# chao1224/GeoSSL

Measured on AMD Instinct MI355X. Metric: molecules/s/GPU SchNet+DDM fwd+bwd (QM9-sized, bs=1024); % HBM roofline, higher is better.
Workload: dtype f32

## Files before the change

### geossl_amd/csrc/ddm.hip

```cpp
#include "common.h"
#include "geossl_hip.h"
#include "tn.h"
#include "wgrad.h"

using namespace geossl;

namespace {

inline int grid1d(int64_t n, int block, int cap = 2048) {
  int64_t g = (n + block - 1) / block;
  return (int)(g < 1 ? 1 : (g > cap ? cap : g));
}

__global__ __launch_bounds__(256) void k_sum_partial(const float* __restrict__ x, int64_t n, float* __restrict__ partial) {
  __shared__ float red[256];
  const int64_t per = (n + gridDim.x - 1) / gridDim.x;
  const int64_t lo = blockIdx.x * per, hi = min(n, lo + per);
  float s = 0.0f;
  for (int64_t i = lo + threadIdx.x; i < hi; i += 256) s += x[i];
  red[threadIdx.x] = s;
  __syncthreads();
  for (int o = 128; o > 0; o >>= 1) {
    if (threadIdx.x < o) red[threadIdx.x] += red[threadIdx.x + o];
    __syncthreads();
  }
  if (threadIdx.x == 0) partial[blockIdx.x] = red[0];
}
__global__ void k_loss_final(const float* __restrict__ partial, int nblk, const int64_t* __restrict__ divisor,
                             float out_scale, float* __restrict__ loss, int accumulate) {
  if (blockIdx.x != 0) return;
  float s = 0.0f;
  for (int b = threadIdx.x; b < nblk; b += 64) s += partial[b];
  s = wave_sum(s);
  if (threadIdx.x != 0) return;
// ... 140 lines not shown
    P[H + F + k] = s_w1;
    P[H + 2 * F + k] = s_b1;
  }
  if (threadIdx.x == 0) {
    float sg = 0.0f, sd = 0.0f;
    for (int s = lo; s < hi; ++s) {
      sg += grow[s];
      sd += demb[s];
    }
    P[H + 3 * F] = sg;
    P[H + 3 * F + 1] = sd;
  }
}
__global__ __launch_bounds__(64) void k_ncsn_small_reduce(const float* __restrict__ partial, int nblk, int F,
                                                          GeosslNcsnGrads g, int accumulate) {
  const int H = F / 2, len = H + 3 * F + 2;
  const int i = blockIdx.x;
  if (i >= len) return;
  float s = 0.0f;
  for (int b = threadIdx.x; b < nblk; b += 64) s += partial[(size_t)b * len + i];
  s = wave_sum(s);
  if (threadIdx.x == 0) {
    float* dst;
    if (i < H) dst = g.o3_w + i;
    else if (i < H + F) dst = g.in_w2 + (i - H);
    else if (i < H + 2 * F) dst = g.in_w1 + (i - H - F);
    else if (i < H + 3 * F) dst = g.in_b1 + (i - H - 2 * F);
    else if (i == H + 3 * F) dst = g.o3_b;
    else dst = g.in_b2;
    *dst = accumulate ? *dst + s : s;
  }
}

__global__ __launch_bounds__(256) void k_incidence_gather(const float* __restrict__ dfeat0,
                                                          const int64_t* __restrict__ inc_ptr,
                                                          const int32_t* __restrict__ inc_idx, int N, int F,
                                                          float* __restrict__ dh0, int accumulate,
                                                          const float* __restrict__ dfeat1, float* __restrict__ dh1,
                                                          const int32_t* __restrict__ dyn_view) {
  const float* __restrict__ dfeat = blockIdx.y == 0 ? dfeat0 : dfeat1;
  float* __restrict__ dh = blockIdx.y == 0 ? dh0 : dh1;
  N = dyn_count(N, dyn_view);
  if (dyn_view != nullptr && blockIdx.y == 1) dh += (size_t)N * F;
  const int per = ((int)gridDim.x + 7) / 8;
  const int grp = ((int)blockIdx.x % 8) * per + (int)blockIdx.x / 8;
  const int a = grp * 4 + (threadIdx.x >> 6), lane = threadIdx.x & 63;
  if (a >= N) return;
  const int64_t p0 = inc_ptr[a], p1 = inc_ptr[a + 1];
  float acc[4] = {0.0f, 0.0f, 0.0f, 0.0f};
  if (accumulate) {
#pragma unroll
    for (int v = 0; v < 4; ++v)
      if (lane + 64 * v < F) acc[v] = dh[(size_t)a * F + lane + 64 * v];
  }
  for (int64_t pb = p0; pb < p1; pb += 64) {
    const int cnt = (int)min((int64_t)64, p1 - pb);
    const int mine = lane < cnt ? inc_idx[pb + lane] : 0;
    for (int q0 = 0; q0 < cnt; q0 += 8) {
      float val[8][4];
#pragma unroll
      for (int u = 0; u < 8; ++u) {
        const int s = __shfl(mine, min(q0 + u, cnt - 1), 64);
#pragma unroll
        for (int v = 0; v < 4; ++v)
          if (lane + 64 * v < F) val[u][v] = dfeat[(size_t)s * F + lane + 64 * v];
      }
#pragma unroll
      for (int u = 0; u < 8; ++u)
        if (q0 + u < cnt) {
#pragma unroll
          for (int v = 0; v < 4; ++v)
            if (lane + 64 * v < F) acc[v] += val[u][v];
        }
    }
  }
#pragma unroll
  for (int v = 0; v < 4; ++v)
    if (lane + 64 * v < F) dh[(size_t)a * F + lane + 64 * v] = acc[v];
}

__global__ void k_adam(float* __restrict__ p, const float* __restrict__ g, float* __restrict__ m,
                       float* __restrict__ v, int64_t n, float step_size, float w1, float beta2, float w2, float eps,
                       float wd, float bc2_sqrt, float grad_scale) {
  for (int64_t i = (int64_t)blockIdx.x * blockDim.x + threadIdx.x; i < n; i += (int64_t)gridDim.x * blockDim.x) {
    float gi = mul_rn(g[i], grad_scale);
    const float pi = p[i];
    if (wd != 0.0f) gi = fmaf(wd, pi, gi);
    const float m0 = m[i];
    const float mi = fmaf(w1, add_rn(gi, -m0), m0);
    const float vi = fmaf(w2, mul_rn(gi, gi), mul_rn(v[i], beta2));
    m[i] = mi;
    v[i] = vi;
    const float denom = add_rn(sqrtf(vi) / bc2_sqrt, eps);
    p[i] = fmaf(-step_size, mi / denom, pi);
  }
}

}

namespace geossl {
int launch_ncsn_small_reduce(const float* partial, int nblk, int F, const GeosslNcsnGrads& g, int accumulate,
                             hipStream_t stream);
}

extern "C" int64_t geossl_loss_reduce_workspace_floats(int64_t S) { return GEOSSL_LOSS_BLOCKS; }

extern "C" int geossl_loss_reduce(const float* loss_e, int64_t S, const int64_t* stats_divisor, float out_scale,
                                  float* loss, float* workspace, int accumulate, hipStream_t stream) {
  hipLaunchKernelGGL(k_sum_partial, dim3(GEOSSL_LOSS_BLOCKS), dim3(256), 0, stream, loss_e, S, workspace);
  GEOSSL_CHECK_LAUNCH();
  hipLaunchKernelGGL(k_loss_final, dim3(1), dim3(64), 0, stream, workspace, GEOSSL_LOSS_BLOCKS, stats_divisor, out_scale,
// ... 47 lines not shown
  NcsnW2Ops l2{grow, w->o3_w, saved->a2, saved->a1, F, H};
  if (F == 128) rc = launch_wgrad_split<2, 4>(l2, 1, S, H, F, o, F, 1, workspace, accumulate, stream);
  else if (F == 64) rc = launch_wgrad_split<1, 2>(l2, 1, S, H, F, o, F, 1, workspace, accumulate, stream);
  else rc = launch_wgrad_split<1, 1>(l2, 1, S, H, F, o, F, 1, workspace, accumulate, stream);
  if (rc) return rc;
  o.dW[0] = grads->o1_w;
  o.db[0] = grads->o1_b;
  o.dd[0] = grads->o1_w + F;
  NcsnW1Ops l1{dz1, h, sei0, sei1, saved->emb, F};
  if (F == 128) rc = launch_wgrad_split<4, 4>(l1, 1, S, F, F, o, F + 1, F + 1, workspace, accumulate, stream);
  else if (F == 64) rc = launch_wgrad_split<2, 2>(l1, 1, S, F, F, o, F + 1, F + 1, workspace, accumulate, stream);
  else rc = launch_wgrad_split<1, 1>(l1, 1, S, F, F, o, F + 1, F + 1, workspace, accumulate, stream);
  if (rc) return rc;
  int chunk, nblk;
  small_plan(S, &chunk, &nblk);
  hipLaunchKernelGGL(k_ncsn_small_partial, dim3(nblk), dim3(128), 0, stream, *w, *saved, grow, demb, (int)S, F, chunk,
                     workspace);
  GEOSSL_CHECK_LAUNCH();
  return launch_ncsn_small_reduce(workspace, nblk, F, *grads, accumulate, stream);
}

namespace geossl {
int launch_ncsn_small_reduce(const float* partial, int nblk, int F, const GeosslNcsnGrads& g, int accumulate,
                             hipStream_t stream) {
  hipLaunchKernelGGL(k_ncsn_small_reduce, dim3(F / 2 + 3 * F + 2), dim3(64), 0, stream, partial, nblk, F, g, accumulate);
  GEOSSL_CHECK_LAUNCH();
  return 0;
}
}

extern "C" int geossl_incidence_gather(const float* dfeat, const int64_t* inc_ptr, const int32_t* inc_idx, int64_t N,
                                       int F, float* dh, int accumulate, hipStream_t stream) {
  if (N <= 0) return 0;
  const unsigned groups = (unsigned)((N + 3) / 4);
  hipLaunchKernelGGL(k_incidence_gather, dim3((groups + 7) / 8 * 8), dim3(256), 0, stream, dfeat, inc_ptr, inc_idx,
                     (int)N, F, dh, accumulate, (const float*)nullptr, (float*)nullptr, (const int32_t*)nullptr);
  GEOSSL_CHECK_LAUNCH();
  return 0;
}

namespace geossl {
int launch_incidence_gather2(const float* dfeat0, const float* dfeat1, const int64_t* inc_ptr, const int32_t* inc_idx,
                             int64_t N, int F, float* dh0, float* dh1, hipStream_t stream, const int32_t* dyn_view) {
  if (N <= 0) return 0;
  const unsigned groups = (unsigned)((N + 3) / 4);
  hipLaunchKernelGGL(k_incidence_gather, dim3((groups + 7) / 8 * 8, 2), dim3(256), 0, stream, dfeat0, inc_ptr, inc_idx,
                     (int)N, F, dh0, 0, dfeat1, dh1, dyn_view);
  GEOSSL_CHECK_LAUNCH();
  return 0;
}
}

extern "C" int geossl_adam_step(float* param, const float* grad, float* exp_avg, float* exp_avg_sq, int64_t n, double lr,
                                double beta1, double beta2, double eps, double weight_decay, int64_t step_count,
                                float grad_scale, hipStream_t stream) {
  if (n <= 0) return 0;
  const double bc1 = 1.0 - pow(beta1, (double)step_count);
  const double bc2 = 1.0 - pow(beta2, (double)step_count);
  hipLaunchKernelGGL(k_adam, dim3(grid1d(n, 256)), dim3(256), 0, stream, param, grad, exp_avg, exp_avg_sq, n,
                     (float)(lr / bc1), (float)(1.0 - beta1), (float)beta2, (float)(1.0 - beta2), (float)eps,
                     (float)weight_decay, (float)sqrt(bc2), grad_scale);
  GEOSSL_CHECK_LAUNCH();
  return 0;
}
```

### geossl_amd/csrc/ncsn_bwd.hip

```cpp
#include "common.h"
#include "geossl_hip.h"
#include "split.h"
#include "tn.h"

using namespace geossl;

namespace {

constexpr int TR = 32;

#ifdef NB_TIMING
__device__ long long nb_dbg[2 * 32 * 8];
#define NB_MARK(slot)                                                                              \
  do {                                                                                             \
    if (blockIdx.x == 5 && lane == 0 && (wave == 0 || wave == NW) && t - t_begin < 32)             \
      nb_dbg[((wave == 0 ? 0 : 1) * 32 + (t - t_begin)) * 8 + (slot)] = clock64();                 \
  } while (0)
#else
#define NB_MARK(slot) do {} while (0)
#endif

template <int NW>
struct NbLds {
  static constexpr int F = 32 * NW, H = F / 2, KHS = (H + 15) / 16, HMB = (H + 31) / 32, KS = F / 16;
  u32x4* zb;
  u32x4* dz2T;
  u32x4* fT;
  u32x4* dz1r;
  u32x4* abT;
  int4* scal;
  float* pdv;
  float* dep;
  float* wls;
  int* eg;
// ... 569 lines not shown
    if (nb < KHS) {
      float* Ps = a.psm + pb * (H + 3 * F + 2);
#pragma unroll
      for (int e = 0; e < 8; ++e) {
        float v = o3acc[e];
#pragma unroll
        for (int o = 16; o > 0; o >>= 1) v += __shfl_xor(v, o, 64);
        const int m = 16 * nb + 8 * kh + e;
        if (j == 0 && m < H) Ps[m] = v;
      }
    }
  }
}

template <int NW>
__global__ __launch_bounds__(128 * NW) void k_ncsn_bwd_fused(NcsnFusedArgs a) {
  if ((int)(threadIdx.x >> 6) < NW) ncsn_bwd_body<NW, true>(a, a.S, a.h);
  else ncsn_bwd_body<NW, false>(a, a.S, a.h);
}
struct NcsnFusedPair { NcsnFusedArgs a[2]; };
template <int NW>
__global__ __launch_bounds__(128 * NW) void k_ncsn_bwd_fused2(NcsnFusedPair pr, const int32_t* __restrict__ dyn_S,
                                                              const int32_t* __restrict__ dyn_view) {
  const NcsnFusedArgs& a = pr.a[blockIdx.y];
  const int S = dyn_count(a.S, dyn_S);
  const float* h = a.h;
  if (dyn_view != nullptr && blockIdx.y == 1) h += (size_t)(*dyn_view) * (32 * NW);
  if ((int)(threadIdx.x >> 6) < NW) ncsn_bwd_body<NW, true>(a, S, h);
  else ncsn_bwd_body<NW, false>(a, S, h);
}

__device__ __forceinline__ void ncsn_reduce_all_block(const ReduceMulti& m, int nblk, int accumulate,
                                                      const float* __restrict__ psm, int F, const GeosslNcsnGrads& g,
                                                      float (*red)[64]) {
  const int mb = m.xoff[m.nseg];
  if ((int)blockIdx.x < mb) {
    reduce_multi_block(m, nblk, accumulate, red, 0);
    return;
  }
  const int H = F / 2, len = H + 3 * F + 2;
  const int i = ((int)blockIdx.x - mb) * 4 + (int)(threadIdx.x >> 6), lane = threadIdx.x & 63;
  if (i >= len) return;
  float s = 0.0f;
  for (int b = lane; b < nblk; b += 64) s += psm[(size_t)b * len + i];
  s = wave_sum(s);
  if (lane == 0) {
    float* dst;
    if (i < H) dst = g.o3_w + i;
    else if (i < H + F) dst = g.in_w2 + (i - H);
    else if (i < H + 2 * F) dst = g.in_w1 + (i - H - F);
    else if (i < H + 3 * F) dst = g.in_b1 + (i - H - 2 * F);
    else if (i == H + 3 * F) dst = g.o3_b;
    else dst = g.in_b2;
    *dst = accumulate ? *dst + s : s;
  }
}
__global__ __launch_bounds__(256) void k_ncsn_reduce_all(ReduceMulti m, int nblk, int accumulate,
                                                         const float* __restrict__ psm, int F, GeosslNcsnGrads g) {
  __shared__ float red[4][64];
  ncsn_reduce_all_block(m, nblk, accumulate, psm, F, g, red);
}
__global__ __launch_bounds__(256) void k_ncsn_reduce_all2(ReduceMulti m0, ReduceMulti m1, int nblk, int accumulate,
                                                          const float* __restrict__ psm0,
                                                          const float* __restrict__ psm1, int F, GeosslNcsnGrads g0,
                                                          GeosslNcsnGrads g1) {
  __shared__ float red[4][64];
  if (blockIdx.y == 0) ncsn_reduce_all_block(m0, nblk, accumulate, psm0, F, g0, red);
  else ncsn_reduce_all_block(m1, nblk, accumulate, psm1, F, g1, red);
}

inline int fused_blocks(int64_t S) {
  const int64_t ntiles = (S + TR - 1) / TR;
  return (int)(ntiles < 256 ? ntiles : 256);
}

}

#ifdef NB_TIMING
extern "C" int geossl_ncsn_bwd_debug_read(long long* host) {
  return (int)hipMemcpyFromSymbol(host, HIP_SYMBOL(nb_dbg), sizeof(long long) * 2 * 32 * 8);
}
#endif

extern "C" int64_t geossl_ddm_loss_bwd_fused_workspace_floats(int64_t S, int F) {
  const int64_t nb = fused_blocks(S), H = F / 2;
  return nb * ((int64_t)F * F + 2 * F + H * F + H + (H + 3 * F + 2));
}

extern "C" int geossl_ddm_loss_bwd_fused(const float* h, const int64_t* sei0, const int64_t* sei1, int64_t S, int64_t N,
                                         int F, const GeosslNcsnWeights* w, const GeosslNcsnSaved* saved,
                                         const int64_t* stats_divisor, float out_scale, const float* gout, float* dfeat,
                                         float* demb, float* grow, const GeosslNcsnGrads* grads, float* workspace,
                                         int accumulate, hipStream_t stream) {
  if (S <= 0) return 0;
  if (F != 32 && F != 64 && F != 128) return (int)hipErrorInvalidValue;
  if (S * (int64_t)F * 4 >= ((int64_t)1 << 32) || N * (int64_t)F * 4 >= ((int64_t)1 << 32)) return (int)hipErrorInvalidValue;
  const int nb = fused_blocks(S), H = F / 2;
  NcsnFusedArgs a;
  a.h = h; a.sei0 = sei0; a.sei1 = sei1; a.S = (int)S; a.w = *w; a.sv = *saved; a.divisor = stats_divisor;
  a.out_scale = out_scale; a.gout = gout; a.dfeat = dfeat; a.demb = demb; a.grow = grow;
  a.pw1 = workspace;
  a.pd1 = a.pw1 + (size_t)nb * F * F;
  a.pb1 = a.pd1 + (size_t)nb * F;
  a.pw2 = a.pb1 + (size_t)nb * F;
  a.pb2 = a.pw2 + (size_t)nb * H * F;
  a.psm = a.pb2 + (size_t)nb * H;
#define LAUNCH(NWV)                                                                                      \
  do {                                                                                                   \
    allow_big_lds(&k_ncsn_bwd_fused<NWV>);                                                               \
    hipLaunchKernelGGL((k_ncsn_bwd_fused<NWV>), dim3(nb), dim3(128 * NWV), NbLds<NWV>::bytes(), stream, a); \
  } while (0)
  if (F == 128) LAUNCH(4); else if (F == 64) LAUNCH(2); else LAUNCH(1);
#undef LAUNCH
  GEOSSL_CHECK_LAUNCH();
  ReduceMulti rm;
  float* o1w[1] = {grads->o1_w};
  float* o1c[1] = {grads->o1_w + F};
  float* o1b[1] = {grads->o1_b};
  float* o2w[1] = {grads->o2_w};
  float* o2b[1] = {grads->o2_b};
  rm.add(a.pw1, F * F, F, F + 1, 1, o1w, 1);
  rm.add(a.pd1, F, F, F, F + 1, o1c, 1);
  rm.add(a.pb1, F, F, F, 1, o1b, 1);
  rm.add(a.pw2, H * F, F, F, 1, o2w, 1);
  rm.add(a.pb2, H, H, H, 1, o2b, 1);
  hipLaunchKernelGGL(k_ncsn_reduce_all, dim3(rm.blocks() + (H + 3 * F + 2 + 3) / 4, 1), dim3(256), 0, stream, rm, nb,
                     accumulate, a.psm, F, *grads);
  GEOSSL_CHECK_LAUNCH();
  return 0;
}

namespace geossl {
int launch_incidence_gather2(const float* dfeat0, const float* dfeat1, const int64_t* inc_ptr, const int32_t* inc_idx,
                             int64_t N, int F, float* dh0, float* dh1, hipStream_t stream, const int32_t* dyn_view);
}

extern "C" int geossl_ddm_loss_bwd_fused2(const GeosslNcsnHeadBwd* heads, const int64_t* sei0, const int64_t* sei1,
                                          int64_t S, int64_t N, int F, const int64_t* stats_divisor, const float* gout,
                                          const int64_t* inc_ptr, const int32_t* inc_idx, int accumulate,
                                          hipStream_t stream) {
  return geossl_ddm_loss_bwd_fused2_dyn(heads, sei0, sei1, S, N, F, stats_divisor, gout, inc_ptr, inc_idx, accumulate,
                                        nullptr, nullptr, stream);
}

extern "C" int geossl_ddm_loss_bwd_fused2_dyn(const GeosslNcsnHeadBwd* heads, const int64_t* sei0, const int64_t* sei1,
                                              int64_t S, int64_t N, int F, const int64_t* stats_divisor,
                                              const float* gout, const int64_t* inc_ptr, const int32_t* inc_idx,
                                              int accumulate, const int32_t* dyn_S, const int32_t* dyn_view,
                                              hipStream_t stream) {
  if (S <= 0) return 0;
  if (heads == nullptr || (F != 32 && F != 64 && F != 128)) return (int)hipErrorInvalidValue;
  if (S * (int64_t)F * 4 >= ((int64_t)1 << 32) || N * (int64_t)F * 4 >= ((int64_t)1 << 32)) return (int)hipErrorInvalidValue;
  const int nb = (fused_blocks(S) + 1) / 2, H = F / 2;
  NcsnFusedPair pr;
  NcsnFusedArgs* a = pr.a;
  for (int k = 0; k < 2; ++k) {
    const GeosslNcsnHeadBwd& hd = heads[k];
    if (hd.h == nullptr || hd.dfeat == nullptr || hd.workspace == nullptr) return (int)hipErrorInvalidValue;
    NcsnFusedArgs& x = a[k];
    x.h = hd.h; x.sei0 = sei0; x.sei1 = sei1; x.S = (int)S; x.w = hd.w; x.sv = hd.saved; x.divisor = stats_divisor;
    x.out_scale = hd.out_scale; x.gout = gout; x.dfeat = hd.dfeat; x.demb = hd.demb; x.grow = hd.grow;
    x.pw1 = hd.workspace;
    x.pd1 = x.pw1 + (size_t)nb * F * F;
    x.pb1 = x.pd1 + (size_t)nb * F;
    x.pw2 = x.pb1 + (size_t)nb * F;
    x.pb2 = x.pw2 + (size_t)nb * H * F;
    x.psm = x.pb2 + (size_t)nb * H;
  }
#define LAUNCH2(NWV)                                                                                                \
  do {                                                                                                              \
    allow_big_lds(&k_ncsn_bwd_fused2<NWV>);                                                                         \
    hipLaunchKernelGGL((k_ncsn_bwd_fused2<NWV>), dim3(nb, 2), dim3(128 * NWV), NbLds<NWV>::bytes(), stream, pr,         \
                       dyn_S, dyn_view);                                                                            \
  } while (0)
  if (F == 128) LAUNCH2(4); else if (F == 64) LAUNCH2(2); else LAUNCH2(1);
#undef LAUNCH2
  GEOSSL_CHECK_LAUNCH();
  ReduceMulti rm[2];
  for (int k = 0; k < 2; ++k) {
    const GeosslNcsnGrads* grads = &heads[k].grads;
    float* o1w[1] = {grads->o1_w};
    float* o1c[1] = {grads->o1_w + F};
    float* o1b[1] = {grads->o1_b};
    float* o2w[1] = {grads->o2_w};
    float* o2b[1] = {grads->o2_b};
    rm[k].add(a[k].pw1, F * F, F, F + 1, 1, o1w, 1);
    rm[k].add(a[k].pd1, F, F, F, F + 1, o1c, 1);
    rm[k].add(a[k].pb1, F, F, F, 1, o1b, 1);
    rm[k].add(a[k].pw2, H * F, F, F, 1, o2w, 1);
    rm[k].add(a[k].pb2, H, H, H, 1, o2b, 1);
  }
  hipLaunchKernelGGL(k_ncsn_reduce_all2, dim3(rm[0].blocks() + (H + 3 * F + 2 + 3) / 4, 2), dim3(256), 0, stream, rm[0],
                     rm[1], nb, accumulate, a[0].psm, a[1].psm, F, heads[0].grads, heads[1].grads);
  GEOSSL_CHECK_LAUNCH();
  if (heads[0].dh != nullptr && heads[1].dh != nullptr)
    return launch_incidence_gather2(heads[0].dfeat, heads[1].dfeat, inc_ptr, inc_idx, N, F, heads[0].dh, heads[1].dh, stream,
                                    dyn_view);
  return 0;
}
```

### geossl_amd/csrc/ncsn_rows.hip

```cpp
#include "common.h"
#include "geossl_hip.h"
#include "split.h"

using namespace geossl;

namespace {

struct RowIn {
  int64_t u, v;
  float sigma, d, eps;
};

template <int NMB>
__device__ __forceinline__ void ncsn_fwd_body(const float* __restrict__ h, const int64_t* __restrict__ batch,
                                              const int64_t* __restrict__ sei0, const int64_t* __restrict__ sei1,
                                              int S, const float* __restrict__ distance,
                                              const int64_t* __restrict__ noise_level,
                                              const float* __restrict__ dist_noise, const GeosslNcsnWeights& w,
                                              float anneal_power, float* __restrict__ loss_e,
                                              const GeosslNcsnSaved& sv, float* __restrict__ loss_part) {
  constexpr int F = 32 * NMB, H = F / 2, HMB = (H + 31) / 32, HP = 32 * HMB, KS = F / 16;
  extern __shared__ __attribute__((aligned(16))) uint8_t smem_raw[];
  u32x4* W1f = reinterpret_cast<u32x4*>(smem_raw);
  u32x4* W2f = W1f + NMB * KS * 3 * 64;
  float* b1s = reinterpret_cast<float*>(W2f + HMB * KS * 3 * 64);
  float* wls = b1s + F;
  float* b2s = wls + F;
  float* w3s = b2s + HP;
  float* iw1 = w3s + HP;
  float* ib1 = iw1 + F;
  float* iw2 = ib1 + F;
  float* lred = iw2 + F;
  const int tid = threadIdx.x, lane = tid & 63, wave = tid >> 6, j = lane & 31, kh = lane >> 5;
  const int nrb = (S + 31) / 32;
  float lsum = 0.0f;
  auto load_row = [&](int rb) {
    RowIn r;
    const int rowc = min(32 * rb + j, S - 1);
    r.u = sei0[rowc];
    r.v = sei1[rowc];
    r.sigma = w.sigmas[noise_level[batch[r.u]]];
    r.d = distance[rowc];
    r.eps = dist_noise[rowc];
    return r;
  };
  int rb = blockIdx.x + gridDim.x * wave;
  RowIn cur;
  if (rb < nrb) cur = load_row(rb);
#ifdef NCSN_STAGE_UNROLL
#pragma unroll
#endif
  for (int i = tid; i < NMB * KS * 64; i += 512) {
    const int ln = i & 63, ks = (i >> 6) % KS, mb = i / (64 * KS);
    const float* row = w.o1_w + (size_t)(32 * mb + (ln & 31)) * (F + 1) + 16 * ks + 8 * (ln >> 5);
    float v[8];
#pragma unroll
    for (int e = 0; e < 8; ++e) v[e] = row[e];
    const Frag3 f = split8(v);
    u32x4* dst = W1f + ((size_t)(mb * KS + ks) * 3) * 64 + ln;
    dst[0] = f.h;
    dst[64] = f.m;
    dst[128] = f.l;
  }
#ifdef NCSN_STAGE_UNROLL
#pragma unroll
#endif
  for (int i = tid; i < HMB * KS * 64; i += 512) {
    const int ln = i & 63, ks = (i >> 6) % KS, mb = i / (64 * KS);
    const int m = 32 * mb + (ln & 31);
    const float* row = w.o2_w + (size_t)min(m, H - 1) * F + 16 * ks + 4 * (ln >> 5);
    const f32x4 lo = *reinterpret_cast<const f32x4*>(row), hi = *reinterpret_cast<const f32x4*>(row + 8);
    float v[8] = {lo.x, lo.y, lo.z, lo.w, hi.x, hi.y, hi.z, hi.w};
    if (m >= H) {
#pragma unroll
      for (int e = 0; e < 8; ++e) v[e] = 0.0f;
    }
    const Frag3 f = split8(v);
    u32x4* dst = W2f + ((size_t)(mb * KS + ks) * 3) * 64 + ln;
    dst[0] = f.h;
    dst[64] = f.m;
    dst[128] = f.l;
  }
  for (int i = tid; i < F; i += 512) {
    b1s[i] = w.o1_b[i];
    wls[i] = w.o1_w[(size_t)i * (F + 1) + F];
    iw1[i] = w.in_w1[i];
    ib1[i] = w.in_b1[i];
    iw2[i] = w.in_w2[i];
  }
  for (int i = tid; i < HP; i += 512) {
    b2s[i] = i < H ? w.o2_b[i] : 0.0f;
    w3s[i] = i < H ? w.o3_w[i] : 0.0f;
  }
  __syncthreads();
  const float ib2 = w.in_b2[0], b3 = w.o3_b[0];
  for (; rb < nrb; rb += gridDim.x * 8) {
    const int row = 32 * rb + j;
    const bool valid = row < S;
    const RowIn in = cur;
    f32x4 gq[2][4];
    auto gather = [&](int ks, f32x4 (&g)[4]) {
      const float* hu = h + (size_t)in.u * F + 16 * ks + 8 * kh;
      const float* hv = h + (size_t)in.v * F + 16 * ks + 8 * kh;
      g[0] = *reinterpret_cast<const f32x4*>(hu);
      g[1] = *reinterpret_cast<const f32x4*>(hu + 4);
      g[2] = *reinterpret_cast<const f32x4*>(hv);
      g[3] = *reinterpret_cast<const f32x4*>(hv + 4);
    };
    gather(0, gq[0]);
    if (rb + gridDim.x * 8 < nrb) cur = load_row(rb + gridDim.x * 8);
    const float pd = add_rn(in.d, mul_rn(in.eps, in.sigma));
    float e = 0.0f;
#pragma unroll 4
    for (int k = kh * (F / 2); k < (kh + 1) * (F / 2); k += 4) {
      const f32x4 a = *reinterpret_cast<const f32x4*>(iw1 + k), b = *reinterpret_cast<const f32x4*>(ib1 + k);
      const f32x4 c = *reinterpret_cast<const f32x4*>(iw2 + k);
      e = fmaf(c.x, fmaxf(fmaf(a.x, pd, b.x), 0.0f), e);
      e = fmaf(c.y, fmaxf(fmaf(a.y, pd, b.y), 0.0f), e);
      e = fmaf(c.z, fmaxf(fmaf(a.z, pd, b.z), 0.0f), e);
      e = fmaf(c.w, fmaxf(fmaf(a.w, pd, b.w), 0.0f), e);
    }
    e += __shfl_xor(e, 32, 64);
    const float emb = e + ib2;
    f32x16 acc1[NMB];
#pragma unroll
    for (int mb = 0; mb < NMB; ++mb)
#pragma unroll
      for (int q = 0; q < 4; ++q) {
        const f32x4 b = *reinterpret_cast<const f32x4*>(b1s + 32 * mb + 8 * q + 4 * kh);
        const f32x4 wl = *reinterpret_cast<const f32x4*>(wls + 32 * mb + 8 * q + 4 * kh);
        acc1[mb][4 * q] = fmaf(emb, wl.x, b.x);
        acc1[mb][4 * q + 1] = fmaf(emb, wl.y, b.y);
        acc1[mb][4 * q + 2] = fmaf(emb, wl.z, b.z);
        acc1[mb][4 * q + 3] = fmaf(emb, wl.w, b.w);
      }
#pragma unroll
    for (int ks = 0; ks < KS; ++ks) {
      if (ks + 1 < KS) gather(ks + 1, gq[(ks + 1) & 1]);
      const f32x4(&g)[4] = gq[ks & 1];
      const float v[8] = {g[0].x + g[2].x, g[0].y + g[2].y, g[0].z + g[2].z, g[0].w + g[2].w,
                          g[1].x + g[3].x, g[1].y + g[3].y, g[1].z + g[3].z, g[1].w + g[3].w};
      const Frag3 bf = split8(v);
      Frag3 af[NMB];
#pragma unroll
      for (int mb = 0; mb < NMB; ++mb) {
        const u32x4* src = W1f + ((size_t)(mb * KS + ks) * 3) * 64 + lane;
        af[mb].h = src[0];
        af[mb].m = src[64];
        af[mb].l = src[128];
      }
#pragma unroll
      for (int mb = 0; mb < NMB; ++mb) acc1[mb] = mfma_bf16(af[mb].l, bf.h, acc1[mb]);
#pragma unroll
      for (int mb = 0; mb < NMB; ++mb) acc1[mb] = mfma_bf16(af[mb].h, bf.l, acc1[mb]);
#pragma unroll
      for (int mb = 0; mb < NMB; ++mb) acc1[mb] = mfma_bf16(af[mb].m, bf.m, acc1[mb]);
#pragma unroll
      for (int mb = 0; mb < NMB; ++mb) acc1[mb] = mfma_bf16(af[mb].m, bf.h, acc1[mb]);
#pragma unroll
      for (int mb = 0; mb < NMB; ++mb) acc1[mb] = mfma_bf16(af[mb].h, bf.m, acc1[mb]);
#pragma unroll
      for (int mb = 0; mb < NMB; ++mb) acc1[mb] = mfma_bf16(af[mb].h, bf.h, acc1[mb]);
      __builtin_amdgcn_sched_barrier(0);
    }
    Frag3 tb[KS];
    {
      float* arow = sv.a1 != nullptr ? sv.a1 + (size_t)row * F + 4 * kh : nullptr;
#pragma unroll
      for (int mb = 0; mb < NMB; ++mb)
#pragma unroll
        for (int half = 0; half < 2; ++half) {
          float v[8];
#pragma unroll
          for (int e2 = 0; e2 < 8; ++e2) v[e2] = fmaxf(acc1[mb][8 * half + e2], 0.0f);
          if (arow != nullptr && valid) {
            *reinterpret_cast<f32x4*>(arow + 32 * mb + 16 * half) = f32x4{v[0], v[1], v[2], v[3]};
            *reinterpret_cast<f32x4*>(arow + 32 * mb + 16 * half + 8) = f32x4{v[4], v[5], v[6], v[7]};
          }
          tb[2 * mb + half] = split8(v);
          __builtin_amdgcn_sched_barrier(0);
        }
    }
    float sc = 0.0f;
#pragma unroll
    for (int mb = 0; mb < HMB; ++mb) {
      f32x16 acc2;
#pragma unroll
      for (int q = 0; q < 4; ++q) {
        const f32x4 b = *reinterpret_cast<const f32x4*>(b2s + 32 * mb + 8 * q + 4 * kh);
        acc2[4 * q] = b.x;
        acc2[4 * q + 1] = b.y;
        acc2[4 * q + 2] = b.z;
        acc2[4 * q + 3] = b.w;
      }
      Frag3 af, an;
      {
        const u32x4* src = W2f + ((size_t)(mb * KS) * 3) * 64 + lane;
        af.h = src[0]; af.m = src[64]; af.l = src[128];
      }
#pragma unroll
      for (int ks = 0; ks < KS; ++ks) {
        if (ks + 1 < KS) {
          const u32x4* src = W2f + ((size_t)(mb * KS + ks + 1) * 3) * 64 + lane;
          an.h = src[0]; an.m = src[64]; an.l = src[128];
        }
        __builtin_amdgcn_sched_barrier(0);
        mma6(acc2, af, tb[ks]);
        __builtin_amdgcn_sched_barrier(0);
        if (ks + 1 < KS) af = an;
      }
      float* a2row = sv.a2 != nullptr ? sv.a2 + (size_t)row * H + 32 * mb + 4 * kh : nullptr;
#pragma unroll
      for (int q = 0; q < 4; ++q) {
        const f32x4 w3 = *reinterpret_cast<const f32x4*>(w3s + 32 * mb + 8 * q + 4 * kh);
        const f32x4 a = f32x4{fmaxf(acc2[4 * q], 0.0f), fmaxf(acc2[4 * q + 1], 0.0f), fmaxf(acc2[4 * q + 2], 0.0f),
                              fmaxf(acc2[4 * q + 3], 0.0f)};
        sc = fmaf(a.x, w3.x, sc);
        sc = fmaf(a.y, w3.y, sc);
        sc = fmaf(a.z, w3.z, sc);
        sc = fmaf(a.w, w3.w, sc);
        if (a2row != nullptr && valid && 32 * mb + 8 * q + 4 * kh < H) *reinterpret_cast<f32x4*>(a2row + 8 * q) = a;
      }
    }
    sc += __shfl_xor(sc, 32, 64);
    const float out = sc + b3;
    const float inv_sigma = 1.0f / in.sigma;
    const float score = out * inv_sigma;
    const float target = (-1.0f / (in.sigma * in.sigma)) * (pd - in.d);
    const float diff = score - target;
    const float pw = powf(in.sigma, anneal_power);
    if (valid && kh == 0) {
      const float le = (0.5f * (diff * diff)) * pw;
      loss_e[row] = le;
      lsum += le;
      if (sv.pd != nullptr) {
        sv.pd[row] = pd;
        sv.emb[row] = emb;
        sv.gscale[row] = diff * pw * inv_sigma;
      }
    }
  }
  if (loss_part != nullptr) {
    lsum = wave_sum(lsum);
    if (lane == 0) lred[wave] = lsum;
    __syncthreads();
    if (tid == 0) {
      float t = 0.0f;
      for (int i = 0; i < 8; ++i) t += lred[i];
      loss_part[blockIdx.x] = t;
    }
    if (blockIdx.x == 0)
      for (int i = (int)gridDim.x + tid; i < GEOSSL_LOSS_PARTIALS; i += 512) loss_part[i] = 0.0f;
  }
}

template <int NMB>
__global__ __launch_bounds__(512) void k_ncsn_fwd(const float* __restrict__ h, const int64_t* __restrict__ batch,
                                                  const int64_t* __restrict__ sei0, const int64_t* __restrict__ sei1,
                                                  int S, const float* __restrict__ distance,
                                                  const int64_t* __restrict__ noise_level,
                                                  const float* __restrict__ dist_noise, GeosslNcsnWeights w,
                                                  float anneal_power, float* __restrict__ loss_e,
                                                  GeosslNcsnSaved sv, float* __restrict__ loss_part) {
  ncsn_fwd_body<NMB>(h, batch, sei0, sei1, S, distance, noise_level, dist_noise, w, anneal_power, loss_e, sv, loss_part);
}
struct NcsnFwdHead {
  const float* h;
  const float* distance;
  const int64_t* noise_level;
  const float* dist_noise;
  GeosslNcsnWeights w;
  GeosslNcsnSaved sv;
  float anneal_power;
// ... 296 lines not shown
```

### geossl_amd/csrc/tn.h

```cpp
#pragma once
#include "common.h"
#include "geossl_hip.h"

namespace geossl {

__global__ void k_reduce_partials(GeosslReduceBatch batch, const float* __restrict__ partial, int nblk, int len,
                                  int ncols, int ld, int cstride, int accumulate);

struct ReduceSeg {
  const float* partial;
  int len, ncols, ld, cstride;
  float* out[GEOSSL_TN_MAX];
};
struct ReduceMulti {
  int nseg;
  int xoff[7];
  ReduceSeg seg[6];
  ReduceMulti() : nseg(0) { xoff[0] = 0; }
  void add(const float* partial, int len, int ncols, int ld, int cstride, float* const* out, int nz) {
    ReduceSeg& g = seg[nseg];
    g.partial = partial;
    g.len = len;
    g.ncols = ncols;
    g.ld = ld;
    g.cstride = cstride;
    for (int z = 0; z < GEOSSL_TN_MAX; ++z) g.out[z] = z < nz ? out[z] : nullptr;
    xoff[nseg + 1] = xoff[nseg] + (len + 63) / 64;
    ++nseg;
  }
  int blocks() const { return xoff[nseg]; }
};
__global__ void k_reduce_multi(ReduceMulti m, int nblk, int accumulate);
__device__ __forceinline__ void reduce_multi_block(const ReduceMulti& m, int nblk, int accumulate, float (*red)[64],
                                                   int z) {
  int g = 0;
  while (g + 1 < m.nseg && (int)blockIdx.x >= m.xoff[g + 1]) ++g;
  const ReduceSeg& sg = m.seg[g];
  float* out = sg.out[z];
  if (out == nullptr) return;
  const int len = sg.len;
  const float* p = sg.partial + (size_t)z * nblk * len;
  const int lane = threadIdx.x & 63, slice = threadIdx.x >> 6;
  const int i = ((int)blockIdx.x - m.xoff[g]) * 64 + lane;
  const int per = (nblk + 3) / 4, b0 = slice * per, b1 = min(nblk, b0 + per);
  float s = 0.0f;
  if (i < len) s = kahan_sum_strided(p + i, b0, b1, len);
  red[slice][lane] = s;
  __syncthreads();
  if (slice == 0 && i < len) {
    const size_t o = (size_t)(i / sg.ncols) * sg.ld + (size_t)(i % sg.ncols) * sg.cstride;
    float v = accumulate ? out[o] : 0.0f;
    v += red[0][lane];
    v += red[1][lane];
    v += red[2][lane];
    v += red[3][lane];
    out[o] = v;
  }
}

inline int64_t tn_workspace_floats(int64_t R, int M, int N, int nprob) {
  int chunk, nblk;
  geossl_tn_plan(R, nprob, &chunk, &nblk);
  return (int64_t)nprob * nblk * ((int64_t)M * N + 2 * M);
}

}
```

Baseline: 421,500.

## Add half-wave incidence gather, fuse gather with reduce, deepen NCSN forward prefetch

Moves the incidence gather into a shared header and adds a specialized F=128 path. In that path each half-wave handles one atom, loads with f32x4 and double-buffers its requests. The dual-head incidence gather is merged into the NCSN reduce-all kernel as extra blocks, which removes one launch and lets the two run concurrently. The NCSN forward kernel gains a configurable gather lookahead and moves next-tile index and sigma loads earlier, interleaved with compute. It also shrinks row indices to int32 and adds fast paths for whole-tile stores. These changes target latency-bound gathers and launch overhead, at the cost of more register pressure from the deeper prefetch buffers.

```diff
diff --git a/geossl_amd/csrc/ddm.hip b/geossl_amd/csrc/ddm.hip
--- a/geossl_amd/csrc/ddm.hip
+++ b/geossl_amd/csrc/ddm.hip
@@ -1,5 +1,6 @@
 #include "common.h"
 #include "geossl_hip.h"
+#include "incidence.h"
 #include "tn.h"
 #include "wgrad.h"
 
@@ -206,51 +207,10 @@
   }
 }
 
-__global__ __launch_bounds__(256) void k_incidence_gather(const float* __restrict__ dfeat0,
-                                                          const int64_t* __restrict__ inc_ptr,
-                                                          const int32_t* __restrict__ inc_idx, int N, int F,
-                                                          float* __restrict__ dh0, int accumulate,
-                                                          const float* __restrict__ dfeat1, float* __restrict__ dh1,
-                                                          const int32_t* __restrict__ dyn_view) {
-  const float* __restrict__ dfeat = blockIdx.y == 0 ? dfeat0 : dfeat1;
-  float* __restrict__ dh = blockIdx.y == 0 ? dh0 : dh1;
-  N = dyn_count(N, dyn_view);
-  if (dyn_view != nullptr && blockIdx.y == 1) dh += (size_t)N * F;
-  const int per = ((int)gridDim.x + 7) / 8;
-  const int grp = ((int)blockIdx.x % 8) * per + (int)blockIdx.x / 8;
-  const int a = grp * 4 + (threadIdx.x >> 6), lane = threadIdx.x & 63;
-  if (a >= N) return;
-  const int64_t p0 = inc_ptr[a], p1 = inc_ptr[a + 1];
-  float acc[4] = {0.0f, 0.0f, 0.0f, 0.0f};
-  if (accumulate) {
-#pragma unroll
-    for (int v = 0; v < 4; ++v)
-      if (lane + 64 * v < F) acc[v] = dh[(size_t)a * F + lane + 64 * v];
-  }
-  for (int64_t pb = p0; pb < p1; pb += 64) {
-    const int cnt = (int)min((int64_t)64, p1 - pb);
-    const int mine = lane < cnt ? inc_idx[pb + lane] : 0;
-    for (int q0 = 0; q0 < cnt; q0 += 8) {
-      float val[8][4];
-#pragma unroll
-      for (int u = 0; u < 8; ++u) {
-        const int s = __shfl(mine, min(q0 + u, cnt - 1), 64);
-#pragma unroll
-        for (int v = 0; v < 4; ++v)
-          if (lane + 64 * v < F) val[u][v] = dfeat[(size_t)s * F + lane + 64 * v];
-      }
-#pragma unroll
-      for (int u = 0; u < 8; ++u)
-        if (q0 + u < cnt) {
-#pragma unroll
-          for (int v = 0; v < 4; ++v)
-            if (lane + 64 * v < F) acc[v] += val[u][v];
-        }
-    }
-  }
-#pragma unroll
-  for (int v = 0; v < 4; ++v)
-    if (lane + 64 * v < F) dh[(size_t)a * F + lane + 64 * v] = acc[v];
+template <bool WIDE>
+__global__ __launch_bounds__(256) void k_incidence_gather(IncidenceArgs g) {
+  if constexpr (WIDE) incidence_gather_block128(g, 0, (int)blockIdx.x, (int)gridDim.x);
+  else incidence_gather_block(g, 0, (int)blockIdx.x, (int)gridDim.x);
 }
 
 __global__ void k_adam(float* __restrict__ p, const float* __restrict__ g, float* __restrict__ m,
@@ -364,23 +324,11 @@
 extern "C" int geossl_incidence_gather(const float* dfeat, const int64_t* inc_ptr, const int32_t* inc_idx, int64_t N,
                                        int F, float* dh, int accumulate, hipStream_t stream) {
   if (N <= 0) return 0;
-  const unsigned groups = (unsigned)((N + 3) / 4);
-  hipLaunchKernelGGL(k_incidence_gather, dim3((groups + 7) / 8 * 8), dim3(256), 0, stream, dfeat, inc_ptr, inc_idx,
-                     (int)N, F, dh, accumulate, (const float*)nullptr, (float*)nullptr, (const int32_t*)nullptr);
-  GEOSSL_CHECK_LAUNCH();
-  return 0;
-}
-
-namespace geossl {
-int launch_incidence_gather2(const float* dfeat0, const float* dfeat1, const int64_t* inc_ptr, const int32_t* inc_idx,
-                             int64_t N, int F, float* dh0, float* dh1, hipStream_t stream, const int32_t* dyn_view) {
-  if (N <= 0) return 0;
-  const unsigned groups = (unsigned)((N + 3) / 4);
-  hipLaunchKernelGGL(k_incidence_gather, dim3((groups + 7) / 8 * 8, 2), dim3(256), 0, stream, dfeat0, inc_ptr, inc_idx,
-                     (int)N, F, dh0, 0, dfeat1, dh1, dyn_view);
-  GEOSSL_CHECK_LAUNCH();
-  return 0;
-}
+  const IncidenceArgs g = {{dfeat, nullptr}, {dh, nullptr}, inc_ptr, inc_idx, nullptr, (int)N, F, accumulate};
+  if (incidence_half_wave(F)) hipLaunchKernelGGL(k_incidence_gather<true>, dim3(incidence_blocks(N, F)), dim3(256), 0, stream, g);
+  else hipLaunchKernelGGL(k_incidence_gather<false>, dim3(incidence_blocks(N, F)), dim3(256), 0, stream, g);
+  GEOSSL_CHECK_LAUNCH();
+  return 0;
 }
 
 extern "C" int geossl_adam_step(float* param, const float* grad, float* exp_avg, float* exp_avg_sq, int64_t n, double lr,
diff --git a/geossl_amd/csrc/incidence.h b/geossl_amd/csrc/incidence.h
--- /dev/null
+++ b/geossl_amd/csrc/incidence.h
@@ -0,0 +1,127 @@
+#pragma once
+#include "common.h"
+
+namespace geossl {
+
+struct IncidenceArgs {
+  const float* dfeat[2];
+  float* dh[2];
+  const int64_t* inc_ptr;
+  const int32_t* inc_idx;
+  const int32_t* dyn_view;
+  int N, F, accumulate;
+};
+
+__device__ __forceinline__ int incidence_group(int bx, int nbx) { return (bx % 8) * ((nbx + 7) / 8) + bx / 8; }
+inline bool incidence_half_wave(int F) {
+#ifdef GEOSSL_INCIDENCE_WAVE_PER_ATOM
+  return false;
+#else
+  return F == 128;
+#endif
+}
+inline unsigned incidence_blocks(int64_t N, int F) {
+  const unsigned groups = (unsigned)(incidence_half_wave(F) ? (N + 7) / 8 : (N + 3) / 4);
+  return (groups + 7) / 8 * 8;
+}
+
+__device__ __forceinline__ void incidence_gather_block(const IncidenceArgs& g, int head, int bx, int nbx) {
+  const float* __restrict__ dfeat = g.dfeat[head];
+  float* __restrict__ dh = g.dh[head];
+  const int N = dyn_count(g.N, g.dyn_view), F = g.F;
+  if (g.dyn_view != nullptr && head == 1) dh += (size_t)N * F;
+  const int a = incidence_group(bx, nbx) * 4 + (threadIdx.x >> 6), lane = threadIdx.x & 63;
+  if (a >= N) return;
+  const int64_t p0 = g.inc_ptr[a], p1 = g.inc_ptr[a + 1];
+  float acc[4] = {0.0f, 0.0f, 0.0f, 0.0f};
+  if (g.accumulate) {
+#pragma unroll
+    for (int v = 0; v < 4; ++v)
+      if (lane + 64 * v < F) acc[v] = dh[(size_t)a * F + lane + 64 * v];
+  }
+  for (int64_t pb = p0; pb < p1; pb += 64) {
+    const int cnt = (int)min((int64_t)64, p1 - pb);
+    const int mine = lane < cnt ? g.inc_idx[pb + lane] : 0;
+    for (int q0 = 0; q0 < cnt; q0 += 8) {
+      float val[8][4];
+#pragma unroll
+      for (int u = 0; u < 8; ++u) {
+        const int s = __shfl(mine, min(q0 + u, cnt - 1), 64);
+#pragma unroll
+        for (int v = 0; v < 4; ++v)
+          if (lane + 64 * v < F) val[u][v] = dfeat[(size_t)s * F + lane + 64 * v];
+      }
+#pragma unroll
+      for (int u = 0; u < 8; ++u)
+        if (q0 + u < cnt) {
+#pragma unroll
+          for (int v = 0; v < 4; ++v)
+            if (lane + 64 * v < F) acc[v] += val[u][v];
+        }
+    }
+  }
+#pragma unroll
+  for (int v = 0; v < 4; ++v)
+    if (lane + 64 * v < F) dh[(size_t)a * F + lane + 64 * v] = acc[v];
+}
+
+__device__ __forceinline__ void incidence_gather_block128(const IncidenceArgs& g, int head, int bx, int nbx) {
+  constexpr int F = 128;
+  const float* __restrict__ dfeat = g.dfeat[head];
+  float* __restrict__ dh = g.dh[head];
+  const int N = dyn_count(g.N, g.dyn_view);
+  if (g.dyn_view != nullptr && head == 1) dh += (size_t)N * F;
+  const int lane = threadIdx.x & 63, hl = lane & 31;
+  const int a = incidence_group(bx, nbx) * 8 + (threadIdx.x >> 5);
+  if ((a & ~1) >= N) return;
+  const bool valid = a < N;
+  const int ac = min(a, N - 1);
+  const int64_t p0 = g.inc_ptr[ac];
+  const int cnt = valid ? (int)(g.inc_ptr[ac + 1] - p0) : 0;
+  const int cntu = __builtin_amdgcn_readfirstlane(max(cnt, __shfl_xor(cnt, 32, 64)));
+  float* out = dh + (size_t)ac * F + 4 * hl;
+  f32x4 acc = {0.0f, 0.0f, 0.0f, 0.0f};
+  if (g.accumulate) acc = *reinterpret_cast<const f32x4*>(out);
+  const int self4 = 4 * (lane & 32);
+  auto ids = [&](int b) {
+    const int64_t pos = p0 + min(b + hl, cnt - 1);
+    return g.inc_idx[pos < 0 ? 0 : pos];
+  };
+  auto request = [&](int mine, int k0, int b, f32x4(&v)[16]) {
+#pragma unroll
+    for (int q = 0; q < 4; ++q)
+      if (b + 4 * q < cntu) {
+#pragma unroll
+        for (int u = 0; u < 4; ++u) {
+          const int s = __builtin_amdgcn_ds_bpermute(self4 + 4 * (k0 + 4 * q + u), mine);
+          v[4 * q + u] = *reinterpret_cast<const f32x4*>(dfeat + (size_t)s * F + 4 * hl);
+        }
+      }
+  };
+  auto add = [&](int b, const f32x4(&v)[16]) {
+#pragma unroll
+    for (int q = 0; q < 4; ++q)
+      if (b + 4 * q < cntu) {
+#pragma unroll
+        for (int u = 0; u < 4; ++u)
+          if (b + 4 * q + u < cnt) acc += v[4 * q + u];
+      }
+  };
+  if (cntu > 0) {
+    f32x4 va[16], vb[16];
+    int mine = ids(0);
+    request(mine, 0, 0, va);
+    for (int b = 0; b < cntu; b += 32) {
+      int nxt = mine;
+      if (b + 32 < cntu) nxt = ids(b + 32);
+      request(mine, 16, b + 16, vb);
+      add(b, va);
+      request(nxt, 0, b + 32, va);
+      add(b + 16, vb);
+      mine = nxt;
+    }
+  }
+  if (valid) *reinterpret_cast<f32x4*>(out) = acc;
+}
+
+}
diff --git a/geossl_amd/csrc/ncsn_bwd.hip b/geossl_amd/csrc/ncsn_bwd.hip
--- a/geossl_amd/csrc/ncsn_bwd.hip
+++ b/geossl_amd/csrc/ncsn_bwd.hip
@@ -1,5 +1,6 @@
 #include "common.h"
 #include "geossl_hip.h"
+#include "incidence.h"
 #include "split.h"
 #include "tn.h"
 
@@ -635,14 +636,14 @@
 
 __device__ __forceinline__ void ncsn_reduce_all_block(const ReduceMulti& m, int nblk, int accumulate,
                                                       const float* __restrict__ psm, int F, const GeosslNcsnGrads& g,
-                                                      float (*red)[64]) {
+                                                      float (*red)[64], int bx) {
   const int mb = m.xoff[m.nseg];
-  if ((int)blockIdx.x < mb) {
-    reduce_multi_block(m, nblk, accumulate, red, 0);
+  if (bx < mb) {
+    reduce_multi_block(m, nblk, accumulate, red, 0, bx);
     return;
   }
   const int H = F / 2, len = H + 3 * F + 2;
-  const int i = ((int)blockIdx.x - mb) * 4 + (int)(threadIdx.x >> 6), lane = threadIdx.x & 63;
+  const int i = (bx - mb) * 4 + (int)(threadIdx.x >> 6), lane = threadIdx.x & 63;
   if (i >= len) return;
   float s = 0.0f;
   for (int b = lane; b < nblk; b += 64) s += psm[(size_t)b * len + i];
@@ -661,15 +662,30 @@
 __global__ __launch_bounds__(256) void k_ncsn_reduce_all(ReduceMulti m, int nblk, int accumulate,
                                                          const float* __restrict__ psm, int F, GeosslNcsnGrads g) {
   __shared__ float red[4][64];
-  ncsn_reduce_all_block(m, nblk, accumulate, psm, F, g, red);
+  ncsn_reduce_all_block(m, nblk, accumulate, psm, F, g, red, (int)blockIdx.x);
 }
 __global__ __launch_bounds__(256) void k_ncsn_reduce_all2(ReduceMulti m0, ReduceMulti m1, int nblk, int accumulate,
                                                           const float* __restrict__ psm0,
                                                           const float* __restrict__ psm1, int F, GeosslNcsnGrads g0,
                                                           GeosslNcsnGrads g1) {
   __shared__ float red[4][64];
-  if (blockIdx.y == 0) ncsn_reduce_all_block(m0, nblk, accumulate, psm0, F, g0, red);
-  else ncsn_reduce_all_block(m1, nblk, accumulate, psm1, F, g1, red);
+  if (blockIdx.y == 0) ncsn_reduce_all_block(m0, nblk, accumulate, psm0, F, g0, red, (int)blockIdx.x);
+  else ncsn_reduce_all_block(m1, nblk, accumulate, psm1, F, g1, red, (int)blockIdx.x);
+}
+template <bool WIDE>
+__global__ __launch_bounds__(256) void k_ncsn_gather_reduce2(ReduceMulti m0, ReduceMulti m1, int nblk, int accumulate,
+                                                             const float* __restrict__ psm0,
+                                                             const float* __restrict__ psm1, int F, GeosslNcsnGrads g0,
+                                                             GeosslNcsnGrads g1, IncidenceArgs ia, int gx) {
+  __shared__ float red[4][64];
+  const int bx = (int)blockIdx.x;
+  if (bx < gx) {
+    if constexpr (WIDE) incidence_gather_block128(ia, (int)blockIdx.y, bx, gx);
+    else incidence_gather_block(ia, (int)blockIdx.y, bx, gx);
+    return;
+  }
+  if (blockIdx.y == 0) ncsn_reduce_all_block(m0, nblk, accumulate, psm0, F, g0, red, bx - gx);
+  else ncsn_reduce_all_block(m1, nblk, accumulate, psm1, F, g1, red, bx - gx);
 }
 
 inline int fused_blocks(int64_t S) {
@@ -733,11 +749,6 @@
   return 0;
 }
 
-namespace geossl {
-int launch_incidence_gather2(const float* dfeat0, const float* dfeat1, const int64_t* inc_ptr, const int32_t* inc_idx,
-                             int64_t N, int F, float* dh0, float* dh1, hipStream_t stream, const int32_t* dyn_view);
-}
-
 extern "C" int geossl_ddm_loss_bwd_fused2(const GeosslNcsnHeadBwd* heads, const int64_t* sei0, const int64_t* sei1,
                                           int64_t S, int64_t N, int F, const int64_t* stats_divisor, const float* gout,
                                           const int64_t* inc_ptr, const int32_t* inc_idx, int accumulate,
@@ -793,11 +804,22 @@
     rm[k].add(a[k].pw2, H * F, F, F, 1, o2w, 1);
     rm[k].add(a[k].pb2, H, H, H, 1, o2b, 1);
   }
-  hipLaunchKernelGGL(k_ncsn_reduce_all2, dim3(rm[0].blocks() + (H + 3 * F + 2 + 3) / 4, 2), dim3(256), 0, stream, rm[0],
-                     rm[1], nb, accumulate, a[0].psm, a[1].psm, F, heads[0].grads, heads[1].grads);
+  const unsigned rblocks = (unsigned)(rm[0].blocks() + (H + 3 * F + 2 + 3) / 4);
+  if (heads[0].dh == nullptr || heads[1].dh == nullptr || N <= 0) {
+    hipLaunchKernelGGL(k_ncsn_reduce_all2, dim3(rblocks, 2), dim3(256), 0, stream, rm[0], rm[1], nb, accumulate, a[0].psm,
+                       a[1].psm, F, heads[0].grads, heads[1].grads);
+    GEOSSL_CHECK_LAUNCH();
+    return 0;
+  }
+  const IncidenceArgs ia = {{heads[0].dfeat, heads[1].dfeat}, {heads[0].dh, heads[1].dh}, inc_ptr, inc_idx, dyn_view,
+                            (int)N, F, 0};
+  const unsigned gx = incidence_blocks(N, F);
+  if (incidence_half_wave(F))
+    hipLaunchKernelGGL(k_ncsn_gather_reduce2<true>, dim3(gx + rblocks, 2), dim3(256), 0, stream, rm[0], rm[1], nb,
+                       accumulate, a[0].psm, a[1].psm, F, heads[0].grads, heads[1].grads, ia, (int)gx);
+  else
+    hipLaunchKernelGGL(k_ncsn_gather_reduce2<false>, dim3(gx + rblocks, 2), dim3(256), 0, stream, rm[0], rm[1], nb,
+                       accumulate, a[0].psm, a[1].psm, F, heads[0].grads, heads[1].grads, ia, (int)gx);
   GEOSSL_CHECK_LAUNCH();
-  if (heads[0].dh != nullptr && heads[1].dh != nullptr)
-    return launch_incidence_gather2(heads[0].dfeat, heads[1].dfeat, inc_ptr, inc_idx, N, F, heads[0].dh, heads[1].dh, stream,
-                                    dyn_view);
   return 0;
 }
diff --git a/geossl_amd/csrc/ncsn_rows.hip b/geossl_amd/csrc/ncsn_rows.hip
--- a/geossl_amd/csrc/ncsn_rows.hip
+++ b/geossl_amd/csrc/ncsn_rows.hip
@@ -7,9 +7,29 @@
 namespace {
 
 struct RowIn {
-  int64_t u, v;
+  int u, v;
   float sigma, d, eps;
 };
+
+#ifndef NCSN_FWD_AHEAD
+#define NCSN_FWD_AHEAD 2
+#endif
+constexpr int kAhead = NCSN_FWD_AHEAD;
+#ifdef NCSN_FWD_NO_PIN
+constexpr bool kPinRequests = false;
+#else
+constexpr bool kPinRequests = true;
+#endif
+#ifdef NCSN_FWD_NO_TILE_START
+constexpr bool kTileStart = false;
+#else
+constexpr bool kTileStart = true;
+#endif
+#ifdef NCSN_FWD_NO_WHOLE_TILES
+constexpr bool kWholeTiles = false;
+#else
+constexpr bool kWholeTiles = true;
+#endif
 
 template <int NMB>
 __device__ __forceinline__ void ncsn_fwd_body(const float* __restrict__ h, const int64_t* __restrict__ batch,
@@ -31,8 +51,10 @@
   float* ib1 = iw1 + F;
   float* iw2 = ib1 + F;
   float* lred = iw2 + F;
-  const int tid = threadIdx.x, lane = tid & 63, wave = tid >> 6, j = lane & 31, kh = lane >> 5;
+  const int tid = threadIdx.x, lane = tid & 63, j = lane & 31, kh = lane >> 5;
+  const int wave = __builtin_amdgcn_readfirstlane(tid >> 6);
   const int nrb = (S + 31) / 32;
+  const bool save_a1 = sv.a1 != nullptr, save_a2 = sv.a2 != nullptr, save_row = sv.pd != nullptr;
   float lsum = 0.0f;
   auto load_row = [&](int rb) {
     RowIn r;
@@ -45,6 +67,7 @@
     return r;
   };
   int rb = blockIdx.x + gridDim.x * wave;
+  const int stride = gridDim.x * 8;
   RowIn cur;
   if (rb < nrb) cur = load_row(rb);
 #ifdef NCSN_STAGE_UNROLL
@@ -94,21 +117,44 @@
   }
   __syncthreads();
   const float ib2 = w.in_b2[0], b3 = w.o3_b[0];
-  for (; rb < nrb; rb += gridDim.x * 8) {
+  f32x4 gq[kAhead + 1][4];
+  auto gather = [&](const RowIn& r, int ks, f32x4 (&g)[4]) {
+    const float* hu = h + (size_t)r.u * F + 16 * ks + 8 * kh;
+    const float* hv = h + (size_t)r.v * F + 16 * ks + 8 * kh;
+    g[0] = *reinterpret_cast<const f32x4*>(hu);
+    g[1] = *reinterpret_cast<const f32x4*>(hu + 4);
+    g[2] = *reinterpret_cast<const f32x4*>(hv);
+    g[3] = *reinterpret_cast<const f32x4*>(hv + 4);
+  };
+  auto gather_head = [&](const RowIn& r) {
+#pragma unroll
+    for (int i = 0; i < kAhead && i < KS; ++i) gather(r, i, gq[i]);
+  };
+  RowIn in = cur;
+  if (kTileStart && rb < nrb) gather_head(in);
+  auto tile = [&]() __attribute__((always_inline)) {
     const int row = 32 * rb + j;
     const bool valid = row < S;
-    const RowIn in = cur;
-    f32x4 gq[2][4];
-    auto gather = [&](int ks, f32x4 (&g)[4]) {
-      const float* hu = h + (size_t)in.u * F + 16 * ks + 8 * kh;
-      const float* hv = h + (size_t)in.v * F + 16 * ks + 8 * kh;
-      g[0] = *reinterpret_cast<const f32x4*>(hu);
-      g[1] = *reinterpret_cast<const f32x4*>(hu + 4);
-      g[2] = *reinterpret_cast<const f32x4*>(hv);
-      g[3] = *reinterpret_cast<const f32x4*>(hv + 4);
+    const bool whole = kWholeTiles && 32 * rb + 32 <= S;
+    auto store_rows = [&](auto&& st) __attribute__((always_inline)) {
+      if (whole) st();
+      else if (valid) st();
     };
-    gather(0, gq[0]);
-    if (rb + gridDim.x * 8 < nrb) cur = load_row(rb + gridDim.x * 8);
+    const bool more = rb + stride < nrb;
+    int lane_t = lane, k4 = 4 * kh;
+    asm volatile("" : "+v"(lane_t), "+v"(k4));
+    if (!kTileStart) {
+      gather_head(in);
+      if (more) cur = load_row(rb + stride);
+    }
+    int64_t mol = 0, lvl = 0;
+    if (kTileStart) {
+      const int rowc = min(32 * (rb + stride) + j, S - 1);
+      cur.u = sei0[rowc];
+      cur.v = sei1[rowc];
+      cur.d = distance[rowc];
+      cur.eps = dist_noise[rowc];
+    }
     const float pd = add_rn(in.d, mul_rn(in.eps, in.sigma));
     float e = 0.0f;
 #pragma unroll 4
@@ -127,8 +173,8 @@
     for (int mb = 0; mb < NMB; ++mb)
 #pragma unroll
       for (int q = 0; q < 4; ++q) {
-        const f32x4 b = *reinterpret_cast<const f32x4*>(b1s + 32 * mb + 8 * q + 4 * kh);
-        const f32x4 wl = *reinterpret_cast<const f32x4*>(wls + 32 * mb + 8 * q + 4 * kh);
+        const f32x4 b = *reinterpret_cast<const f32x4*>(b1s + 32 * mb + 8 * q + k4);
+        const f32x4 wl = *reinterpret_cast<const f32x4*>(wls + 32 * mb + 8 * q + k4);
         acc1[mb][4 * q] = fmaf(emb, wl.x, b.x);
         acc1[mb][4 * q + 1] = fmaf(emb, wl.y, b.y);
         acc1[mb][4 * q + 2] = fmaf(emb, wl.z, b.z);
@@ -136,15 +182,21 @@
       }
 #pragma unroll
     for (int ks = 0; ks < KS; ++ks) {
-      if (ks + 1 < KS) gather(ks + 1, gq[(ks + 1) & 1]);
-      const f32x4(&g)[4] = gq[ks & 1];
+      if (ks + kAhead < KS) gather(in, ks + kAhead, gq[(ks + kAhead) % (kAhead + 1)]);
+      if (kTileStart) {
+        if (ks == KS / 4) mol = batch[cur.u];
+        if (ks == KS / 2) lvl = noise_level[mol];
+        if (ks == 3 * KS / 4) cur.sigma = w.sigmas[lvl];
+      }
+      if (kPinRequests) __builtin_amdgcn_sched_barrier(0);
+      const f32x4(&g)[4] = gq[ks % (kAhead + 1)];
       const float v[8] = {g[0].x + g[2].x, g[0].y + g[2].y, g[0].z + g[2].z, g[0].w + g[2].w,
                           g[1].x + g[3].x, g[1].y + g[3].y, g[1].z + g[3].z, g[1].w + g[3].w};
       const Frag3 bf = split8(v);
       Frag3 af[NMB];
 #pragma unroll
       for (int mb = 0; mb < NMB; ++mb) {
-        const u32x4* src = W1f + ((size_t)(mb * KS + ks) * 3) * 64 + lane;
+        const u32x4* src = W1f + ((size_t)(mb * KS + ks) * 3) * 64 + lane_t;
         af[mb].h = src[0];
         af[mb].m = src[64];
         af[mb].l = src[128];
@@ -165,7 +217,7 @@
     }
     Frag3 tb[KS];
     {
-      float* arow = sv.a1 != nullptr ? sv.a1 + (size_t)row * F + 4 * kh : nullptr;
+      float* arow = save_a1 ? sv.a1 + (size_t)row * F + 4 * kh : nullptr;
 #pragma unroll
       for (int mb = 0; mb < NMB; ++mb)
 #pragma unroll
@@ -173,53 +225,58 @@
           float v[8];
 #pragma unroll
           for (int e2 = 0; e2 < 8; ++e2) v[e2] = fmaxf(acc1[mb][8 * half + e2], 0.0f);
-          if (arow != nullptr && valid) {
-            *reinterpret_cast<f32x4*>(arow + 32 * mb + 16 * half) = f32x4{v[0], v[1], v[2], v[3]};
-            *reinterpret_cast<f32x4*>(arow + 32 * mb + 16 * half + 8) = f32x4{v[4], v[5], v[6], v[7]};
-          }
+          if (save_a1)
+            store_rows([&] {
+              *reinterpret_cast<f32x4*>(arow + 32 * mb + 16 * half) = f32x4{v[0], v[1], v[2], v[3]};
+              *reinterpret_cast<f32x4*>(arow + 32 * mb + 16 * half + 8) = f32x4{v[4], v[5], v[6], v[7]};
+            });
           tb[2 * mb + half] = split8(v);
           __builtin_amdgcn_sched_barrier(0);
         }
     }
-    float sc = 0.0f;
+    f32x16 acc2[HMB];
 #pragma unroll
     for (int mb = 0; mb < HMB; ++mb) {
-      f32x16 acc2;
 #pragma unroll
       for (int q = 0; q < 4; ++q) {
-        const f32x4 b = *reinterpret_cast<const f32x4*>(b2s + 32 * mb + 8 * q + 4 * kh);
-        acc2[4 * q] = b.x;
-        acc2[4 * q + 1] = b.y;
-        acc2[4 * q + 2] = b.z;
-        acc2[4 * q + 3] = b.w;
+        const f32x4 b = *reinterpret_cast<const f32x4*>(b2s + 32 * mb + 8 * q + k4);
+        acc2[mb][4 * q] = b.x;
+        acc2[mb][4 * q + 1] = b.y;
+        acc2[mb][4 * q + 2] = b.z;
+        acc2[mb][4 * q + 3] = b.w;
       }
       Frag3 af, an;
       {
-        const u32x4* src = W2f + ((size_t)(mb * KS) * 3) * 64 + lane;
+        const u32x4* src = W2f + ((size_t)(mb * KS) * 3) * 64 + lane_t;
         af.h = src[0]; af.m = src[64]; af.l = src[128];
       }
 #pragma unroll
       for (int ks = 0; ks < KS; ++ks) {
         if (ks + 1 < KS) {
-          const u32x4* src = W2f + ((size_t)(mb * KS + ks + 1) * 3) * 64 + lane;
+          const u32x4* src = W2f + ((size_t)(mb * KS + ks + 1) * 3) * 64 + lane_t;
           an.h = src[0]; an.m = src[64]; an.l = src[128];
         }
         __builtin_amdgcn_sched_barrier(0);
-        mma6(acc2, af, tb[ks]);
+        mma6(acc2[mb], af, tb[ks]);
         __builtin_amdgcn_sched_barrier(0);
         if (ks + 1 < KS) af = an;
       }
-      float* a2row = sv.a2 != nullptr ? sv.a2 + (size_t)row * H + 32 * mb + 4 * kh : nullptr;
+    }
+    if (kTileStart) gather_head(cur);
+    float sc = 0.0f;
+#pragma unroll
+    for (int mb = 0; mb < HMB; ++mb) {
+      float* a2row = save_a2 ? sv.a2 + (size_t)row * H + 32 * mb + 4 * kh : nullptr;
 #pragma unroll
       for (int q = 0; q < 4; ++q) {
-        const f32x4 w3 = *reinterpret_cast<const f32x4*>(w3s + 32 * mb + 8 * q + 4 * kh);
-        const f32x4 a = f32x4{fmaxf(acc2[4 * q], 0.0f), fmaxf(acc2[4 * q + 1], 0.0f), fmaxf(acc2[4 * q + 2], 0.0f),
-                              fmaxf(acc2[4 * q + 3], 0.0f)};
+        const f32x4 w3 = *reinterpret_cast<const f32x4*>(w3s + 32 * mb + 8 * q + k4);
+        const f32x4 a = f32x4{fmaxf(acc2[mb][4 * q], 0.0f), fmaxf(acc2[mb][4 * q + 1], 0.0f),
+                              fmaxf(acc2[mb][4 * q + 2], 0.0f), fmaxf(acc2[mb][4 * q + 3], 0.0f)};
         sc = fmaf(a.x, w3.x, sc);
         sc = fmaf(a.y, w3.y, sc);
         sc = fmaf(a.z, w3.z, sc);
         sc = fmaf(a.w, w3.w, sc);
-        if (a2row != nullptr && valid && 32 * mb + 8 * q + 4 * kh < H) *reinterpret_cast<f32x4*>(a2row + 8 * q) = a;
+        if (save_a2 && 32 * mb + 8 * q + 4 * kh < H) store_rows([&] { *reinterpret_cast<f32x4*>(a2row + 8 * q) = a; });
       }
     }
     sc += __shfl_xor(sc, 32, 64);
@@ -233,12 +290,16 @@
       const float le = (0.5f * (diff * diff)) * pw;
       loss_e[row] = le;
       lsum += le;
-      if (sv.pd != nullptr) {
+      if (save_row) {
         sv.pd[row] = pd;
         sv.emb[row] = emb;
         sv.gscale[row] = diff * pw * inv_sigma;
       }
     }
+    in = cur;
+  };
+  for (; rb < nrb; rb += stride) {
+    tile();
   }
   if (loss_part != nullptr) {
     lsum = wave_sum(lsum);
diff --git a/geossl_amd/csrc/tn.h b/geossl_amd/csrc/tn.h
--- a/geossl_amd/csrc/tn.h
+++ b/geossl_amd/csrc/tn.h
@@ -32,16 +32,16 @@
 };
 __global__ void k_reduce_multi(ReduceMulti m, int nblk, int accumulate);
 __device__ __forceinline__ void reduce_multi_block(const ReduceMulti& m, int nblk, int accumulate, float (*red)[64],
-                                                   int z) {
+                                                   int z, int bx) {
   int g = 0;
-  while (g + 1 < m.nseg && (int)blockIdx.x >= m.xoff[g + 1]) ++g;
+  while (g + 1 < m.nseg && bx >= m.xoff[g + 1]) ++g;
   const ReduceSeg& sg = m.seg[g];
   float* out = sg.out[z];
   if (out == nullptr) return;
   const int len = sg.len;
   const float* p = sg.partial + (size_t)z * nblk * len;
   const int lane = threadIdx.x & 63, slice = threadIdx.x >> 6;
-  const int i = ((int)blockIdx.x - m.xoff[g]) * 64 + lane;
+  const int i = (bx - m.xoff[g]) * 64 + lane;
   const int per = (nblk + 3) / 4, b0 = slice * per, b1 = min(nblk, b0 + per);
   float s = 0.0f;
   if (i < len) s = kahan_sum_strided(p + i, b0, b1, len);
@@ -58,6 +58,11 @@
   }
 }
 
+__device__ __forceinline__ void reduce_multi_block(const ReduceMulti& m, int nblk, int accumulate, float (*red)[64],
+                                                   int z) {
+  reduce_multi_block(m, nblk, accumulate, red, z, (int)blockIdx.x);
+}
+
 inline int64_t tn_workspace_floats(int64_t R, int M, int N, int nprob) {
   int chunk, nblk;
   geossl_tn_plan(R, nprob, &chunk, &nblk);
```

Result: no change. 421,500 (-0.0%).
